# synsense/HaghighatshoarMuir2024

Measured on AMD Instinct MI355X. Metric: audio samples/sec through STHT+RZCC+SNN beamform, 7-mic 48kHz 360-DoA; DoA MAE vs ref, higher is better.
Workload: dtype f64

## Files before the change

haghighatshoarmuir2024_amd/csrc/beamform_lean.hip:

```cpp
#include "micloc_internal.h"

namespace micloc {

namespace {

typedef double double4_t __attribute__((ext_vector_type(4)));
typedef double double2_t __attribute__((ext_vector_type(2)));
typedef unsigned uint2_t __attribute__((ext_vector_type(2)));

constexpr int LEAN_THREADS = BF_WAVES * 64;
constexpr int LEAN_NT = 2;
constexpr int LEAN_CH = BF_WAVES * LEAN_NT * 16;
constexpr int LEAN_TILES = LEAN_CH / 16;
constexpr int LEAN_C = 14;
constexpr int LEAN_KM = 3, LEAN_KV = 2;

__device__ __forceinline__ void lean_chunk_order(int &chunk, int &b)
{
    const int nchunks = gridDim.x, nb = gridDim.y;
    const int L = chunk + nchunks * b;
    const int full = (nb >> 3) << 3;
    if (L < full * nchunks) {
        const int j = L >> 3;
        const int bq = j / nchunks;
        chunk = j - bq * nchunks;
        b = 8 * bq + (L & 7);
    }
}

__device__ __forceinline__ double lean_row_sum4(double x)
{
    unsigned lo = __double2loint(x), hi = __double2hiint(x);
    uint2_t a = __builtin_amdgcn_permlane16_swap(lo, lo, false, false);
    uint2_t b = __builtin_amdgcn_permlane16_swap(hi, hi, false, false);
    const double s = __hiloint2double(b[0], a[0]) + __hiloint2double(b[1], a[1]);
    lo = __double2loint(s);
    hi = __double2hiint(s);
    a = __builtin_amdgcn_permlane32_swap(lo, lo, false, false);
    b = __builtin_amdgcn_permlane32_swap(hi, hi, false, false);
    return __hiloint2double(b[0], a[0]) + __hiloint2double(b[1], a[1]);
}

__device__ __forceinline__ double lean_row_sum4_pair(double a, double b)
{
    uint2_t lo = __builtin_amdgcn_permlane16_swap(__double2loint(a), __double2loint(b), false, false);
    uint2_t hi = __builtin_amdgcn_permlane16_swap(__double2hiint(a), __double2hiint(b), false, false);
    const double s = __hiloint2double(hi[0], lo[0]) + __hiloint2double(hi[1], lo[1]);
    const unsigned sl = __double2loint(s), sh = __double2hiint(s);
    lo = __builtin_amdgcn_permlane32_swap(sl, sl, false, false);
    hi = __builtin_amdgcn_permlane32_swap(sh, sh, false, false);
    return __hiloint2double(hi[0], lo[0]) + __hiloint2double(hi[1], lo[1]);
}

template <int NG>
__device__ __forceinline__ void lean_stage2(const double *Vl, const double *__restrict__ Wp, int Gp, int wv, int l, int ntile,
                                            double *__restrict__ pout)
{
    const int lc = l & 15;
    const int q = l >> 4;
    double Wf[NG][LEAN_KM], Wv[NG][LEAN_KV];
    const unsigned of = (unsigned)(q * Gp + lc), ov = (unsigned)lc;
#pragma unroll
    for (int j = 0; j < NG; ++j) {
        const double *wp = Wp + 16 * (wv + BF_WAVES * j);
#pragma unroll
        for (int k = 0; k < LEAN_KM; ++k) Wf[j][k] = (wp + (size_t)(4 * k) * Gp)[of];
#pragma unroll
        for (int i = 0; i < LEAN_KV; ++i) Wv[j][i] = (wp + (size_t)(4 * LEAN_KM + i) * Gp)[ov];
    }
    double sq[NG];
#pragma unroll
    for (int j = 0; j < NG; ++j) sq[j] = 0.0;
    const double *pf = Vl + l;
    const double *pt = Vl + 64 * LEAN_KM + q;
    auto tile_step = [&](const int tile) {
        double V[LEAN_KM];
#pragma unroll
        for (int k = 0; k < LEAN_KM; ++k) V[k] = pf[256 * tile + 64 * k];
        double4_t acc[NG];
#pragma unroll
        for (int k = 0; k < LEAN_KM; ++k)
#pragma unroll
            for (int j = 0; j < NG; ++j)
                acc[j] = __builtin_amdgcn_mfma_f64_16x16x4f64(V[k], Wf[j][k], k == 0 ? double4_t{0.0, 0.0, 0.0, 0.0} : acc[j], 0, 0, 0);
#pragma unroll
        for (int i = 0; i < LEAN_KV; ++i) {
            double Vv[4];
#pragma unroll
            for (int r = 0; r < 4; ++r) Vv[r] = pt[256 * tile + 16 * i + 4 * r];
#pragma unroll
            for (int j = 0; j < NG; ++j)
#pragma unroll
                for (int r = 0; r < 4; ++r) acc[j][r] = __builtin_fma(Vv[r], Wv[j][i], acc[j][r]);
        }
#pragma unroll
        for (int r = 0; r < 4; ++r)
#pragma unroll
            for (int j = 0; j < NG; ++j) sq[j] = __builtin_fma(acc[j][r], acc[j][r], sq[j]);
    };
#pragma unroll 1
    for (int t = 0; t < ntile; ++t) tile_step(t);
    if constexpr (NG >= 2) {
        const double s = lean_row_sum4_pair(sq[0], sq[1]);
        if (l < 32) pout[16 * (wv + BF_WAVES * q) + lc] = s;
    } else {
        const double s = lean_row_sum4(sq[0]);
        if (l < 16) pout[16 * wv + l] = s;
    }
    if constexpr (NG == 3) {
        const double s = lean_row_sum4(sq[2]);
        if (l < 16) pout[16 * (wv + BF_WAVES * 2) + l] = s;
    }
}

}

template <int NK, int NGW>
__global__ __launch_bounds__(LEAN_THREADS, 6) void beamform_ws_kernel_lean(const int8_t *__restrict__ spikes, const double *__restrict__ ntab_g,
                                                                            const double *__restrict__ Wp, int GT, int T,
                                                                            double *__restrict__ partial)
{
    constexpr int R = LEAN_CH + 4 * NK - 16;
    constexpr int NTAB = 4 * NK + 16;
    constexpr int NB8 = R * LEAN_C / 8;
    static_assert(R * 16 >= LEAN_TILES * 256, "the parked fragments alias the spike tile");
    static_assert((R * LEAN_C) % 8 == 0 && 4 * NB8 < 13000, "wide staging: whole 8-byte words, and the division by 7 below");
    __shared__ __attribute__((aligned(16))) double smem[R * 16 + NTAB];
    double *S = smem;
    double *Vl = smem;
    double *ntab = smem + R * 16;
    const int Gp = 16 * GT;
    const int tid = threadIdx.x;
    const int wv = __builtin_amdgcn_readfirstlane(tid >> 6);
    const int l = tid & 63;
    const int lc = l & 15;
    const int q = l >> 4;
    int chunk = blockIdx.x, b = blockIdx.y;
    lean_chunk_order(chunk, b);
    const int nchunks = gridDim.x;
    const int cs = chunk * LEAN_CH;

    for (int e = tid; e < NTAB; e += LEAN_THREADS) ntab[e] = ntab_g[e];
    {
        const int8_t *sb = spikes + (size_t)b * T * LEAN_C;
        const int tau0 = cs + 16 - 4 * NK;
        if (tau0 >= 0 && tau0 + R <= T) {
            const int8_t *src = sb + (size_t)tau0 * LEAN_C;
            for (int i = tid; i < NB8; i += LEAN_THREADS) {
                uint2_t w;
                __builtin_memcpy(&w, src + 8 * i, 8);
                const int row0 = (4 * i * 9363) >> 16;
                const int col0 = 8 * i - LEAN_C * row0;
                const int k = (LEAN_C - col0) >> 1;
                double *d = S + row0 * 16 + col0;
#pragma unroll
                for (int p = 0; p < 4; ++p) {
                    const unsigned h = w[p >> 1] >> (16 * (p & 1));
                    double2_t v;
                    v[0] = (double)(int)(int8_t)(h & 0xff);
                    v[1] = (double)(int)(int8_t)((h >> 8) & 0xff);
                    double *dp = (p > 0 && p >= k) ? d + 2 : d;
                    *reinterpret_cast<double2_t *>(dp + 2 * p) = v;
                }
            }
            for (int rho = tid; rho < R; rho += LEAN_THREADS) *reinterpret_cast<double2_t *>(S + rho * 16 + LEAN_C) = double2_t{0.0, 0.0};
        } else {
            const int c = tid & 15;
            constexpr int RP = LEAN_THREADS / 16;
            const int rr = tid >> 4;
            if (c >= LEAN_C) {
                for (int rho = rr; rho < R; rho += RP) S[rho * 16 + c] = 0.0;
            } else {
                for (int r0 = rr; r0 < R; r0 += RP * 6) {
                    int8_t v[6];
#pragma unroll
                    for (int i = 0; i < 6; ++i) {
                        int tau = tau0 + r0 + RP * i;
                        tau = tau < 0 ? 0 : (tau >= T ? T - 1 : tau);
                        v[i] = sb[(size_t)tau * LEAN_C + c];
                    }
#pragma unroll
                    for (int i = 0; i < 6; ++i) {
                        const int rho = r0 + RP * i;
                        const int tau = tau0 + rho;
                        if (rho < R) S[rho * 16 + c] = (tau >= 0 && tau < T) ? (double)v[i] : 0.0;
                    }
                }
            }
        }
    }
    __syncthreads();

    const int tb0 = cs + wv * LEAN_NT * 16;
    const bool active = tb0 < T;
    double4_t vacc[LEAN_NT];
    if (active) {
        const double *sp = S + (wv * LEAN_NT * 16 + q) * 16 + lc;
        const double *np_ = ntab + (lc - q + 3);
#pragma unroll
        for (int ks = 0; ks < NK; ++ks) {
            const double bn = np_[4 * (NK - 1 - ks)];
            double a[LEAN_NT];
#pragma unroll
            for (int tt = 0; tt < LEAN_NT; ++tt) a[tt] = sp[(16 * tt + 4 * ks) * 16];
#pragma unroll
            for (int tt = 0; tt < LEAN_NT; ++tt)
                vacc[tt] = __builtin_amdgcn_mfma_f64_16x16x4f64(a[tt], bn, ks == 0 ? double4_t{0.0, 0.0, 0.0, 0.0} : vacc[tt], 0, 0, 0);
        }
    }
    __syncthreads();
    if (active) {
        if (tb0 + LEAN_NT * 16 > T) {
#pragma unroll
            for (int tt = 0; tt < LEAN_NT; ++tt) {
                const bool tvalid = (tb0 + 16 * tt + lc) < T;
#pragma unroll
                for (int r = 0; r < 4; ++r) vacc[tt][r] = tvalid ? vacc[tt][r] : 0.0;
            }
        }
#pragma unroll
        for (int tt = 0; tt < LEAN_NT; ++tt) {
            double *vp = Vl + (wv * LEAN_NT + tt) * 256 + l;
#pragma unroll
            for (int r = 0; r < 4; ++r) vp[64 * r] = vacc[tt][r];
        }
    }
    __syncthreads();

    int ntile = (T - cs + 15) >> 4;
    ntile = ntile > LEAN_TILES ? LEAN_TILES : ntile;
    double *pout = partial + ((size_t)b * nchunks + chunk) * Gp;
    const bool owns_all = wv + BF_WAVES * (NGW - 1) < GT;
    if (owns_all)
        lean_stage2<NGW>(Vl, Wp, Gp, wv, l, ntile, pout);
    else
        lean_stage2<NGW - 1>(Vl, Wp, Gp, wv, l, ntile, pout);
}

bool launch_lif_beamform_lean(const BeamformW &W, const NeuronTab &nt, const int8_t *spikes, int B, int T, double *y, double *partial,
                              hipStream_t stream, int *nchunks, hipError_t *err)
{
    if (VARIANT_WS_GENERAL_ONLY) return false;
    if (y || !partial || W.chunk_range || W.complex_pairs || W.CT != 1 || W.C != LEAN_C) return false;
    if ((W.GT + BF_WAVES - 1) / BF_WAVES != 3) return false;
    const int nch = (T + LEAN_CH - 1) / LEAN_CH;
    const dim3 grid(nch, B), block(LEAN_THREADS);
    switch (nt.NK) {
        case 13:
            hipLaunchKernelGGL((beamform_ws_kernel_lean<13, 3>), grid, block, 0, stream, spikes, nt.tab, W.Wp, W.GT, T, partial);
            break;
        default: return false;
    }
    *nchunks = nch;
    *err = hipGetLastError();
    return true;
}

}
```

Before: 3.723 billion.

## Fuse stage-2 tail FMAs into inline DPP row-broadcast asm with re-parked LDS tail

Replaces the per-tile scalar tail (loading 8 LDS values for the two extra K rows and doing plain FMAs) with one inline-asm block using v_fmac_f64 with DPP row_newbcast, so each lane loads a single tail value and broadcasts it across rows. The stage-1 LDS store re-parks the fourth accumulator row in a permuted layout to match the broadcast pattern, and the LDS pointer is advanced inside the asm. This cuts LDS reads per tile and the related address arithmetic. The cost is hand-written s_nop hazard padding, fragile asm register constraints, and opaque scheduling around the MFMA results.

Result: no change. 3.734 billion (median of 6 runs) (+0.3%).

```diff
diff --git a/haghighatshoarmuir2024_amd/csrc/beamform_lean.hip b/haghighatshoarmuir2024_amd/csrc/beamform_lean.hip
--- a/haghighatshoarmuir2024_amd/csrc/beamform_lean.hip
+++ b/haghighatshoarmuir2024_amd/csrc/beamform_lean.hip
@@ -52,6 +52,42 @@
     return __hiloint2double(hi[0], lo[0]) + __hiloint2double(hi[1], lo[1]);
 }
 
+#define LEAN_TAIL_FMA(j, r, i, m) "v_fmac_f64_dpp %[a" #j #r "], %[x], %[w" #j #i "] row_newbcast:" #m " row_mask:0xf bank_mask:0xf\n\t"
+#define LEAN_SQ_FMA(j, r) "v_fmac_f64_e32 %[s" #j "], %[a" #j #r "], %[a" #j #r "]\n\t"
+#define LEAN_ACC_OPS(j) [a##j##0] "v"(acc[j][0]), [a##j##1] "v"(acc[j][1]), [a##j##2] "v"(acc[j][2]), [a##j##3] "v"(acc[j][3])
+#define LEAN_ROW2(M, r, i, m) M(0, r, i, m) M(1, r, i, m)
+#define LEAN_ROW3(M, r, i, m) M(0, r, i, m) M(1, r, i, m) M(2, r, i, m)
+#define LEAN_TAIL_RUN(ROW)                                                                                                \
+    "s_nop 15\n\ts_nop 1\n\t"                                                                                            \
+    ROW(LEAN_TAIL_FMA, 0, 0, 0) ROW(LEAN_TAIL_FMA, 1, 0, 1) ROW(LEAN_TAIL_FMA, 2, 0, 2) ROW(LEAN_TAIL_FMA, 3, 0, 3)       \
+    ROW(LEAN_TAIL_FMA, 0, 1, 4) ROW(LEAN_TAIL_FMA, 1, 1, 5) ROW(LEAN_TAIL_FMA, 2, 1, 6) ROW(LEAN_TAIL_FMA, 3, 1, 7)       \
+    ROW(LEAN_SQ, 0, , ) ROW(LEAN_SQ, 1, , ) ROW(LEAN_SQ, 2, , ) ROW(LEAN_SQ, 3, , )                                       \
+    "v_add_u32_e32 %[p], 0x800, %[p]"
+#define LEAN_SQ(j, r, i, m) LEAN_SQ_FMA(j, r)
+
+template <int NG>
+__device__ __forceinline__ void lean_vector_run(const double4_t (&acc)[NG], double (&sq)[NG], const double (&Wv)[NG][LEAN_KV], double x, unsigned &p)
+{
+    static_assert(NG == 2 || NG == 3, "one statement per tile count");
+    if constexpr (NG == 3) {
+        asm volatile(LEAN_TAIL_RUN(LEAN_ROW3)
+                     : [s0] "+v"(sq[0]), [s1] "+v"(sq[1]), [s2] "+v"(sq[2]), [p] "+v"(p)
+                     : LEAN_ACC_OPS(0), LEAN_ACC_OPS(1), LEAN_ACC_OPS(2), [x] "v"(x), [w00] "v"(Wv[0][0]), [w01] "v"(Wv[0][1]),
+                       [w10] "v"(Wv[1][0]), [w11] "v"(Wv[1][1]), [w20] "v"(Wv[2][0]), [w21] "v"(Wv[2][1]));
+    } else {
+        asm volatile(LEAN_TAIL_RUN(LEAN_ROW2)
+                     : [s0] "+v"(sq[0]), [s1] "+v"(sq[1]), [p] "+v"(p)
+                     : LEAN_ACC_OPS(0), LEAN_ACC_OPS(1), [x] "v"(x), [w00] "v"(Wv[0][0]), [w01] "v"(Wv[0][1]), [w10] "v"(Wv[1][0]),
+                       [w11] "v"(Wv[1][1]));
+    }
+}
+
+__device__ __forceinline__ int lean_park_tail(int l)
+{
+    const int lc = l & 15, q = l >> 4;
+    return 16 * (lc & 3) + 4 * q + (lc >> 2);
+}
+
 template <int NG>
 __device__ __forceinline__ void lean_stage2(const double *Vl, const double *__restrict__ Wp, int Gp, int wv, int l, int ntile,
                                             double *__restrict__ pout)
@@ -71,35 +107,22 @@
     double sq[NG];
 #pragma unroll
     for (int j = 0; j < NG; ++j) sq[j] = 0.0;
-    const double *pf = Vl + l;
-    const double *pt = Vl + 64 * LEAN_KM + q;
-    auto tile_step = [&](const int tile) {
-        double V[LEAN_KM];
-#pragma unroll
-        for (int k = 0; k < LEAN_KM; ++k) V[k] = pf[256 * tile + 64 * k];
+    unsigned p = 8u * (unsigned)l;
+    auto frag = [&](const int k) { return *reinterpret_cast<const double *>(reinterpret_cast<const char *>(Vl) + p + 8 * 64 * k); };
+    auto tile_step = [&]() {
+        const double x = frag(LEAN_KM);
+        const double v0 = frag(0), v1 = frag(1), v2 = frag(2);
         double4_t acc[NG];
 #pragma unroll
-        for (int k = 0; k < LEAN_KM; ++k)
-#pragma unroll
-            for (int j = 0; j < NG; ++j)
-                acc[j] = __builtin_amdgcn_mfma_f64_16x16x4f64(V[k], Wf[j][k], k == 0 ? double4_t{0.0, 0.0, 0.0, 0.0} : acc[j], 0, 0, 0);
-#pragma unroll
-        for (int i = 0; i < LEAN_KV; ++i) {
-            double Vv[4];
-#pragma unroll
-            for (int r = 0; r < 4; ++r) Vv[r] = pt[256 * tile + 16 * i + 4 * r];
-#pragma unroll
-            for (int j = 0; j < NG; ++j)
-#pragma unroll
-                for (int r = 0; r < 4; ++r) acc[j][r] = __builtin_fma(Vv[r], Wv[j][i], acc[j][r]);
-        }
-#pragma unroll
-        for (int r = 0; r < 4; ++r)
-#pragma unroll
-            for (int j = 0; j < NG; ++j) sq[j] = __builtin_fma(acc[j][r], acc[j][r], sq[j]);
+        for (int j = 0; j < NG; ++j) acc[j] = __builtin_amdgcn_mfma_f64_16x16x4f64(v0, Wf[j][0], double4_t{0.0, 0.0, 0.0, 0.0}, 0, 0, 0);
+#pragma unroll
+        for (int j = 0; j < NG; ++j) acc[j] = __builtin_amdgcn_mfma_f64_16x16x4f64(v1, Wf[j][1], acc[j], 0, 0, 0);
+#pragma unroll
+        for (int j = 0; j < NG; ++j) acc[j] = __builtin_amdgcn_mfma_f64_16x16x4f64(v2, Wf[j][2], acc[j], 0, 0, 0);
+        lean_vector_run<NG>(acc, sq, Wv, x, p);
     };
 #pragma unroll 1
-    for (int t = 0; t < ntile; ++t) tile_step(t);
+    for (int t = 0; t < ntile; ++t) tile_step();
     if constexpr (NG >= 2) {
         const double s = lean_row_sum4_pair(sq[0], sq[1]);
         if (l < 32) pout[16 * (wv + BF_WAVES * q) + lc] = s;
@@ -220,9 +243,10 @@
         }
 #pragma unroll
         for (int tt = 0; tt < LEAN_NT; ++tt) {
-            double *vp = Vl + (wv * LEAN_NT + tt) * 256 + l;
-#pragma unroll
-            for (int r = 0; r < 4; ++r) vp[64 * r] = vacc[tt][r];
+            double *vp = Vl + (wv * LEAN_NT + tt) * 256;
+#pragma unroll
+            for (int r = 0; r < LEAN_KM; ++r) vp[64 * r + l] = vacc[tt][r];
+            vp[64 * LEAN_KM + lean_park_tail(l)] = vacc[tt][LEAN_KM];
         }
     }
     __syncthreads();
```
